# JuliaRobotics/KernelDensityEstimate.jl

Hardware: AMD Instinct MI355X
Metric: gibbs_product_samples_per_sec (higher is better)
Workload: dtype f64

## Files before the change

### kerneldensityestimate.jl_amd/csrc/gibbs_lean.hip

```cpp
#define KDEHIP_EXP256 1
#ifndef KDEHIP_PRELOAD_MAXB
#define KDEHIP_PRELOAD_MAXB 8
#endif
#include "gibbs_device.hpp"
#include "screen_device.hpp"

namespace kdehip {

template <int I> using IC = std::integral_constant<int, I>;
template <int N, int I = 0, typename F>
__device__ __forceinline__ void static_for(F &&f) {
  if constexpr (I < N) {
    f(IC<I>{});
    static_for<N, I + 1>(f);
  }
}

#if defined(KDEHIP_LEAN_HI) || (defined(KDEHIP_LEAN_DEV_M) && KDEHIP_LEAN_DEV_M > 4)
constexpr int kLeanMinDens = 8, kLeanMaxDens = 8;
#else
constexpr int kLeanMinDens = 2, kLeanMaxDens = 4;
#endif
constexpr int kLeanMaxNormals = 128;

__device__ __forceinline__ int scalar_copy(int x) {
  int y;
  asm("s_mov_b32 %0, %1" : "=s"(y) : "s"(x));
  return y;
}

template <int D>
struct LeanTile {
  int n;
  int flags;
  int lds_off;
  int stage_bytes;
  int chunk_rows;
  int seg;
  int hdr_lo, hdr_hi;
  int B, F, last_lane;
  int uniform_bw;
  __device__ __forceinline__ int64_t hdr_off() const {
    return (static_cast<int64_t>(hdr_hi) << 32) | static_cast<uint32_t>(hdr_lo);
  }
  __device__ __forceinline__ void load(const kdehip_v8i &d) {
    n = scalar_copy(d[0]);
    flags = scalar_copy(d[1]);
    lds_off = scalar_copy(d[2]);
    stage_bytes = scalar_copy(d[3]);
    chunk_rows = scalar_copy(d[4]);
    seg = scalar_copy(d[5]);
    hdr_lo = scalar_copy(d[6]);
    hdr_hi = scalar_copy(d[7]);
    B = (n + 63) >> 6;
    last_lane = flags & 0xFF;
    uniform_bw = flags >> 8;
    F = uniform_bw ? D + 1 : 2 * D + 1;
  }
};

template <typename P, typename T, bool OK> constexpr bool kCanPreloadImpl = OK && kIsLdsPtr<P> && sizeof(T) == 8;

template <typename T, int D, int M, int WAVES, bool BATCH = false, bool SCHUNK = false>
__global__ __launch_bounds__(WAVES * 64) void gibbs_lean_kernel(PlanDev plan_, RunArgs a_) {
  const LaunchView<BATCH> view(plan_, a_);
  const PlanDev &plan = view.plan;
  const auto &a = view.a;
  constexpr bool kPrefetchRows = (WAVES <= 12) || sizeof(T) == 4 || D <= 4;
  using RowPtr = std::conditional_t<(WAVES == 16 && sizeof(T) == 8), LdsPtrSplit<T>, LdsPtr<T>>;
  constexpr int kCopyWaves = WAVES > 4 ? 4 : WAVES;
  constexpr bool kKeptRows = (WAVES <= 8);
  constexpr bool kScreen = sizeof(T) == 8 && !BATCH;
  constexpr bool kPreloadBuild = kKeptRows && kPrefetchRows;
  constexpr int kNormOff = 2048;
  constexpr int kUnifOff = kNormOff + WAVES * kLeanMaxNormals * 8;
  constexpr int kPoolOff = kUnifOff + WAVES * 1024;
  constexpr bool kCoop = kScreen && SCHUNK && WAVES == 8;
  constexpr int kXchgOff = kPoolOff + kLdsPoolBytes;
  constexpr int kXchgSlotDoubles = 32 + 4 * 64;
  constexpr int kXchgBytes = kCoop ? 64 + WAVES * kXchgSlotDoubles * 8 : 0;
  static_assert(kPoolOff + kLdsPoolBytes + kXchgBytes <= 160 * 1024, "LDS budget of one CU exceeded");
  __shared__ __attribute__((aligned(1024))) unsigned char smem[kPoolOff + kLdsPoolBytes + kXchgBytes];

  double *sExpTab = reinterpret_cast<double *>(smem);
  if (threadIdx.x < 256) sExpTab[threadIdx.x] = kExp2Tab256[threadIdx.x];
  if constexpr (kCoop) {
    if (threadIdx.x < 16) reinterpret_cast<int *>(smem + kXchgOff)[threadIdx.x] = 0;
  }

  const int lane = threadIdx.x & 63;
  const int wave = __builtin_amdgcn_readfirstlane(static_cast<int>(threadIdx.x >> 6));
  KDEHIP_PRIO_CHAIN();
  const int chain = wave;
  int64_t s = static_cast<int64_t>(view.block) * WAVES + chain;
  const bool live = s < a.Np;
  if (!live) s = a.Np - 1;
  const uint64_t gs = static_cast<uint64_t>(a.sample_offset + s);
  const void *fb = live ? static_cast<const void *>(plan.levels) : nullptr;

  const int L = plan.L;
  const T *__restrict__ data = static_cast<const T *>(plan.data);
  const LevelTable levels{(const __attribute__((address_space(4))) kdehip_v16i *)(plan.levels)};
  const StepTable steps{(const __attribute__((address_space(4))) kdehip_v8i *)(plan.levels + 2 * plan.M * (plan.L + 1))};
  unsigned char *pool = smem + kPoolOff;
  const int dl = lane < D ? lane : D - 1;
  const int vlev = a.variant % 1000;

  double *sNorm = reinterpret_cast<double *>(smem + kNormOff) + chain * kLeanMaxNormals;
  const int R = D * (L + 1);
  if (a.rng_philox) {
    for (int b = lane; 2 * b < R; b += 64) {
      double n0, n1;
      philox_normal_pair(a.seed, gs, static_cast<uint32_t>(b), n0, n1);
      sNorm[2 * b] = n0;
      if (2 * b + 1 < R) sNorm[2 * b + 1] = n1;
    }
  } else {
    for (int r = lane; r < R; r += 64) sNorm[r] = a.randN[s * a.R + r];
  }
  __syncthreads();

  T lam[M], lmu[M];
  int psel[M];

  auto adopt = [&](auto jc, const auto &ds, auto hdr, int pos) {
    constexpr int j = decltype(jc)::value;
    using TA = TileAddr<T>;
    auto e = hdr + kTileHeader + TA::row(pos >> 6, TA::stride(ds.F)) + (pos & 63) * TA::kLane;
    const T mu = e[dl * TA::kField];
    const T var = ds.uniform_bw ? hdr[dl] : e[(D + dl) * TA::kField];
    const T l = fast_rcp(var);
    lam[j] = l;
    lmu[j] = mu * l;
    psel[j] = pos;
  };
  auto product = [&](auto skipc, T &mean, T &cov) {
    constexpr int skip = decltype(skipc)::value;
    T ls = T(0), ms = T(0);
    static_for<M>([&](auto kc) {
      constexpr int k = decltype(kc)::value;
      if constexpr (k != skip) { ls += lam[k]; ms += lmu[k]; }
    });
    cov = fast_rcp(ls);
    mean = cov * ms;
  };

  auto draw = [&](const auto &ds, auto hdr, T mean, T cov, auto &&run) -> int {
    if (ds.uniform_bw) {
      EvalUniform<T, D> ev;
      ev.tab = sExpTab;
      const T c = hdr[dl] + cov;
      T cen, nin;
      EvalUniform<T, D>::operands(mean, c, true, cen, nin);
      T Pr = T(1);
#pragma unroll
      for (int d = 0; d < D; ++d) {
        ev.center[d] = lane_read(cen, d);
        ev.ninv[d] = lane_read(nin, d);
        Pr *= lane_read(c, d);
      }
      ev.scale = Num<T>::rsqrt(Pr);
      return run(ev);
    }
    EvalFast<T, D, false> ev;
    ev.tab = sExpTab;
    ev.act = 0;
#pragma unroll
    for (int d = 0; d < D; ++d) {
      ev.center[d] = lane_read(mean, d);
      ev.cov[d] = lane_read(cov, d);
    }
    return run(ev);
  };

  uint32_t c = static_cast<uint32_t>(M);
  uint32_t ubatch = 0xFFFFFFFFu;
  double *sUnif = reinterpret_cast<double *>(smem + kUnifOff) + wave * 128;
  auto next_uniform = [&]() -> double {
    const uint32_t b = c >> 7;
    if (b != ubatch) {
      ubatch = b;
      double u_even, u_odd;
      if (a.rng_philox) {
        const Philox4 r = philox_block(a.seed, gs, b * 64u + static_cast<uint32_t>(lane), 0u);
        u_even = bits_to_unit(r.v[0], r.v[1]);
        u_odd = bits_to_unit(r.v[2], r.v[3]);
      } else {
        const int64_t i0 = s * a.K + static_cast<int64_t>(b) * 128 + 2 * lane - 1;
        u_even = (i0 >= 0 && i0 < a.nU) ? a.randU[i0] : 0.5;
        u_odd = (i0 + 1 < a.nU) ? a.randU[i0 + 1] : 0.5;
      }
      wave_sync();
      sUnif[2 * lane] = u_even;
      sUnif[2 * lane + 1] = u_odd;
      wave_sync();
    }
    const double u = sUnif[c & 127u];
    ++c;
    return u;
  };

  static_for<M>([&](auto jc) {
    const LevelDesc ds = levels[decltype(jc)::value * (L + 1)];
    adopt(jc, ds, data + ds.hdr_off, 0);
  });

  const TabTable tabs{(const __attribute__((address_space(4))) kdehip_v8i *)(plan.tabdesc)};
  const T *tables = static_cast<const T *>(plan.tables);
  const int Lt = (vlev == 1 || vlev == 4 || !a.use_tables) ? 0 : plan.Lt;

  auto draw_rows = [&](const auto &ds, auto rows, const auto &ev, double u) -> int {
    using P = decltype(rows);
    return draw_label<T, P, kPrefetchRows, kKeptRows>(rows, ds, lane, ev, u, fb);
  };

  auto draw_rows_repeat = [&](const auto &ds, const T *rows, const auto &ev, double u) -> int {
    using Ev = std::decay_t<decltype(ev)>;
    if constexpr (kScreen && SCHUNK && sizeof(typename Ev::Row) <= 7 * sizeof(T) && WAVES <= 8) {
      LaneAcc<T> acc;
      KDEHIP_PRIO_ROWS();
      lane_rows_all_deep<T, Ev>(rows, ds.B, TileAddr<T>::stride(ds.F), lane, ev, acc);
      KDEHIP_PRIO_CHAIN();
      return select_or_raise<T, const T *>(acc.total(), rows, ds, lane, ev, u, fb);
    }
    return draw_rows(ds, rows, ev, u);
  };

#ifdef KDEHIP_SCREEN_STAMPS
  unsigned long long rstamp[8] = {0, 0, 0, 0, 0, 0, 0, 0}, r_prev_end = 0;
  bool rstamp_on = false;
#define RSTAMP(var) const unsigned long long var = __builtin_amdgcn_s_memtime()
#define RSTAMP_ADD(slot, t0, t1) do { if (rstamp_on) rstamp[slot] += (t1) - (t0); } while (0)
#else
#define RSTAMP(var) do {} while (0)
#define RSTAMP_ADD(slot, t0, t1) do {} while (0)
#endif
  auto step_kept = [&](auto jc, const auto &ds, auto hdr, const auto &row, T mean, T cov, double u) {
    RSTAMP(tr1);
    auto rows1 = hdr + kTileHeader;
    using P1 = decltype(rows1);
    using Ev = EvalFast<T, D, false>;
    Ev ev;
    ev.tab = sExpTab;
    ev.act = 0;
#pragma unroll
    for (int d = 0; d < D; ++d) {
      ev.center[d] = lane_read(mean, d);
      ev.cov[d] = lane_read(cov, d);
    }
#ifdef KDEHIP_SCREEN_STAMPS
    asm volatile("" ::"s"(ev.center[D - 1]), "s"(ev.cov[D - 1]));
#endif
    RSTAMP(tr2);
    RSTAMP_ADD(1, tr1, tr2);
    int pos1;
    if (ds.B == 1) {
      const T S = ev(row);
      pos1 = select_or_raise<T, P1>(S, rows1, ds, lane, ev, u, fb);
    } else if (ds.B <= 4) {
      pos1 = draw_label_kept<T, P1, Ev, 4>(rows1, ds, lane, ev, u, fb, row);
    } else {
      pos1 = draw_label_kept<T, P1, Ev, 8>(rows1, ds, lane, ev, u, fb, row);
    }
    pos1 = __builtin_amdgcn_readfirstlane(pos1);
    RSTAMP(tr3);
    RSTAMP_ADD(2, tr2, tr3);
    adopt(jc, ds, hdr, pos1);
#ifdef KDEHIP_SCREEN_STAMPS
    {
      const double sink = lam[decltype(jc)::value] + lmu[decltype(jc)::value];
      asm volatile("" ::"v"(sink));
    }
#endif
    RSTAMP(tr4);
    RSTAMP_ADD(3, tr3, tr4);
#ifdef KDEHIP_SCREEN_STAMPS
    r_prev_end = tr4;
#endif
  };

  auto step = [&](auto jc, const auto &ds, auto hdr, bool first, T x) {
    if constexpr (kCanPreloadImpl<decltype(hdr + kTileHeader), T, kPreloadBuild>) {
      if (!ds.uniform_bw && ds.B <= KDEHIP_PRELOAD_MAXB) {
        RSTAMP(tr0);
#ifdef KDEHIP_SCREEN_STAMPS
        if (r_prev_end) RSTAMP_ADD(4, r_prev_end, tr0);
#endif
        const auto row = EvalFast<T, D, false>().load(hdr + kTileHeader + lane * TileAddr<T>::kLane);
        T mean1 = x, cov1 = T(0);
        if (!first) product(jc, mean1, cov1);
        const double u1 = next_uniform();
#ifdef KDEHIP_SCREEN_STAMPS
        asm volatile("" ::"v"(mean1), "v"(cov1), "v"(u1));
        {
          RSTAMP(trp);
          RSTAMP_ADD(0, tr0, trp);
        }
#endif
        step_kept(jc, ds, hdr, row, mean1, cov1, u1);
        return;
      }
    }
    T mean = x, cov = T(0);
    if (!first) product(jc, mean, cov);
    const double u = next_uniform();
    auto rows = hdr + kTileHeader;
    const int pos = __builtin_amdgcn_readfirstlane(draw(ds, hdr, mean, cov, [&](const auto &ev) {
      return draw_rows(ds, rows, ev, u);
    }));
    adopt(jc, ds, hdr, pos);
  };

  uint32_t n_screened = 0, n_repeated = 0;
#ifdef KDEHIP_SCREEN_STAMPS
  unsigned long long sstamp[8] = {0, 0, 0, 0, 0, 0, 0, 0};
  bool sstamp_on = false;
#endif
  auto screen_eval = [&](const auto &ds, double mu0, double cmin, float mmax, float valid, T mean, T cov, auto &&body) -> int {
    const float cen = static_cast<float>(mean - mu0);
    const float cf = static_cast<float>(cmin + cov), covf = static_cast<float>(cov);
    const float acen = fabsf(cen);
    const float t = fminf(mmax + acen, 2.0f * acen);
    float a2 = lane < D ? t * t * __builtin_amdgcn_rcpf(cf) : 0.0f;
    const bool inr = (acen <= kScreenMaxAbsMean) && (covf <= static_cast<float>(kScreenMaxVar)) && (a2 <= kScreenMaxA2);
    const bool ok = valid != 0.0f && __ballot(lane < D && !inr) == 0ull;
    if (ds.uniform_bw) {
      ScreenEval<D, true> ev;
      ev.a2 = a2; ev.nsum = (ds.B + 1) >> 1;
      const float ninv = -kScreenC0 * __builtin_amdgcn_rcpf(cf);
      float pr = 1.0f;
#pragma unroll
      for (int d = 0; d < D; ++d) {
        ev.cen[d] = lane_read(cen, d);
        ev.b[d] = lane_read(ninv, d);
        pr *= lane_read(cf, d);
      }
      ev.scale = __builtin_amdgcn_rsqf(pr);
      return body(ev, ok);
    } else {
      ScreenEval<D, false> ev;
      ev.a2 = a2; ev.nsum = (ds.B + 1) >> 1; ev.scale = 1.0f;
#pragma unroll
      for (int d = 0; d < D; ++d) {
        ev.cen[d] = lane_read(cen, d);
        ev.b[d] = lane_read(covf, d);
      }
      return body(ev, ok);
    }
  };
  auto screen_finish = [&](auto jc, const auto &ds, int pos, T mean, T cov, double u) {
    const T *hdrg = data + ds.hdr_off();
    ++n_screened;
    if (pos < 0) {
      ++n_repeated;
      pos = __builtin_amdgcn_readfirstlane(draw(ds, hdrg, mean, cov, [&](const auto &ev) {
        return draw_rows_repeat(ds, hdrg + kTileHeader, ev, u);
      }));
    }
    adopt(jc, ds, hdrg, pos);
  };
  bool pend = false;
  T pend_mean = T(0), pend_cov = T(0);
  double pend_u = 0.0;
  int cstep = 0;
  auto coop_post = [&](T mean, T cov, double u) {
    if constexpr (kCoop) {
      pend = true; pend_mean = mean; pend_cov = cov; pend_u = u;
      double *xs = reinterpret_cast<double *>(smem + kXchgOff + 64) + wave * kXchgSlotDoubles;
      if (lane < D) { xs[dl] = static_cast<double>(mean); xs[8 + dl] = static_cast<double>(cov); }
      if (lane == 0) reinterpret_cast<int *>(smem + kXchgOff)[(cstep & 1) * WAVES + wave] = 1;
    }
  };
  auto coop_resolve = [&](auto jp, const auto &dsp, int par) {
    if constexpr (kCoop) {
      int *flags = reinterpret_cast<int *>(smem + kXchgOff) + par * WAVES;
      const int f = flags[lane & (WAVES - 1)];
      const unsigned mask = static_cast<unsigned>(__ballot(f != 0 && lane < WAVES));
      if (mask == 0u) return;
      using TA = TileAddr<T>;
      const T *hdrg = data + dsp.hdr_off();
      const T *rows = hdrg + kTileHeader;
      const int RS = TA::stride(dsp.F), B = dsp.B;
      const int group = wave >> 2, k = wave & 3;
      int idx = 0;
      for (unsigned m = mask; m != 0u; m &= m - 1u, ++idx) {
        if ((idx & 1) != group) continue;
        const int r = __builtin_ctz(m);
        double *xs = reinterpret_cast<double *>(smem + kXchgOff + 64) + r * kXchgSlotDoubles;
        const T mean_r = static_cast<T>(xs[dl]), cov_r = static_cast<T>(xs[8 + dl]);
        T acc = T(0);
        KDEHIP_PRIO_ROWS();
        draw(dsp, hdrg, mean_r, cov_r, [&](const auto &ev) {
          using Ev = std::decay_t<decltype(ev)>;
          using Row = typename Ev::Row;
          const T *e = rows + lane * TA::kLane;
          auto at = [&](int rr) { return e + TA::row(rr < B ? rr : B - 1, RS); };
          if constexpr (sizeof(Row) <= 4 * sizeof(T)) {
            Row a0 = ev.load(at(k)), a1 = ev.load(at(k + 4)), a2 = ev.load(at(k + 8)), a3 = ev.load(at(k + 12));
            int i = k;
            for (; i + 12 < B; i += 16) {
              const Row b0 = ev.load(at(i + 16)), b1 = ev.load(at(i + 20)), b2 = ev.load(at(i + 24)), b3 = ev.load(at(i + 28));
              __builtin_amdgcn_sched_barrier(0);
              acc += ev(a0); acc += ev(a1); acc += ev(a2); acc += ev(a3);
              a0 = b0; a1 = b1; a2 = b2; a3 = b3;
            }
            if (i < B) acc += ev(a0);
            if (i + 4 < B) acc += ev(a1);
            if (i + 8 < B) acc += ev(a2);
          } else {
            Row a0 = ev.load(at(k)), a1 = ev.load(at(k + 4));
            int i = k;
            for (; i + 4 < B; i += 8) {
              const Row b0 = ev.load(at(i + 8)), b1 = ev.load(at(i + 12));
              __builtin_amdgcn_sched_barrier(0);
              acc += ev(a0); acc += ev(a1);
              a0 = b0; a1 = b1;
            }
            if (i < B) acc += ev(a0);
          }
          return 0;
        });
        KDEHIP_PRIO_CHAIN();
        xs[32 + 64 * k + lane] = static_cast<double>(acc);
      }
      __syncthreads();
      if (pend) {
        double *xs = reinterpret_cast<double *>(smem + kXchgOff + 64) + wave * kXchgSlotDoubles;
        const T a0 = static_cast<T>(xs[32 + lane]), a1 = static_cast<T>(xs[32 + 64 + lane]);
        const T a2 = static_cast<T>(xs[32 + 128 + lane]), a3 = static_cast<T>(xs[32 + 192 + lane]);
        const T S = (a0 + a1) + (a2 + a3);
        const int pos = __builtin_amdgcn_readfirstlane(draw(dsp, hdrg, pend_mean, pend_cov, [&](const auto &ev) {
          return select_or_raise<T, const T *>(S, rows, dsp, lane, ev, pend_u, fb);
        }));
        adopt(jp, dsp, hdrg, pos);
        pend = false;
        if (lane == 0) flags[wave] = 0;
      }
    }
  };

  auto step_screen = [&](auto jc, const auto &ds, int sc_lds_off, bool first, T x) {
    if constexpr (kScreen) {
      SSTAMP(ts0);
      const LdsPtr<float> h32 = (LdsPtr<float>)(pool + sc_lds_off);
      const LdsPtr<double> h64 = (LdsPtr<double>)(pool + sc_lds_off);
      const double mu0 = h64[dl], cmin = h64[8 + dl];
      const float mmax = h32[32 + dl], valid = h32[40];
      T mean = x, cov = T(0);
      if (!first) product(jc, mean, cov);
      const double u = next_uniform();
      SSTAMP(ts1);
      SSTAMP_ADD(0, ts0, ts1);
      const float cen = static_cast<float>(mean - mu0);
      const float cf = static_cast<float>(cmin + cov), covf = static_cast<float>(cov);
      const float acen = fabsf(cen);
      const float t = fminf(mmax + acen, 2.0f * acen);
      float a2 = lane < D ? t * t * __builtin_amdgcn_rcpf(cf) : 0.0f;
      const bool inr = (acen <= kScreenMaxAbsMean) && (covf <= static_cast<float>(kScreenMaxVar)) && (a2 <= kScreenMaxA2);
      int pos = -1;
      const T *hdrg = data + ds.hdr_off();
      if (valid != 0.0f && __ballot(lane < D && !inr) == 0ull) {
        const LdsPtr<float> rows32 = h32 + kScreenHeaderFloats;
        if (ds.uniform_bw) {
          ScreenEval<D, true> ev;
          ev.a2 = a2; ev.nsum = (ds.B + 1) >> 1;
          const float ninv = -kScreenC0 * __builtin_amdgcn_rcpf(cf);
          float pr = 1.0f;
#pragma unroll
          for (int d = 0; d < D; ++d) {
            ev.cen[d] = lane_read(cen, d);
            ev.b[d] = lane_read(ninv, d);
            pr *= lane_read(cf, d);
          }
          ev.scale = __builtin_amdgcn_rsqf(pr);
          pos = screen_draw<D, true>(rows32, ds.n, ds.B, ds.F, lane, ev, u SSTAMP_ARGS);
        } else {
          ScreenEval<D, false> ev;
          ev.a2 = a2; ev.nsum = (ds.B + 1) >> 1; ev.scale = 1.0f;
#pragma unroll
          for (int d = 0; d < D; ++d) {
            ev.cen[d] = lane_read(cen, d);
            ev.b[d] = lane_read(covf, d);
          }
          pos = screen_draw<D, false>(rows32, ds.n, ds.B, ds.F, lane, ev, u SSTAMP_ARGS);
        }
        pos = __builtin_amdgcn_readfirstlane(pos);
      }
      SSTAMP(ts2);
      SSTAMP_ADD(1, ts1, ts2);
      ++n_screened;
      if (pos < 0) {
        ++n_repeated;
        pos = __builtin_amdgcn_readfirstlane(draw(ds, hdrg, mean, cov, [&](const auto &ev) {
          return draw_rows_repeat(ds, hdrg + kTileHeader, ev, u);
        }));
      }
      SSTAMP(ts3);
      SSTAMP_ADD(2, ts2, ts3);
      adopt(jc, ds, hdrg, pos);
#ifdef KDEHIP_SCREEN_STAMPS
      {
        const double sink = lam[decltype(jc)::value] + lmu[decltype(jc)::value];
        asm volatile("" ::"v"(sink));
      }
#endif
      SSTAMP(ts4);
      SSTAMP_ADD(3, ts3, ts4);
    }
  };

  int gchunk = 0;
  auto stage_chunk = [&](const auto &ds, int r0, int half) {
    using TA = TileAddr<T>;
    const int RS = TA::stride(ds.F), rc = ds.chunk_rows;
    const int nrows = (ds.B - r0 < rc) ? (ds.B - r0) : rc;
    const int bytes = (static_cast<int>(TA::span(nrows, RS)) * int(sizeof(T)) + 1023) & ~1023;
    const unsigned char *src = reinterpret_cast<const unsigned char *>(data + ds.hdr_off() + kTileHeader + TA::row(r0, RS));
    if (wave < kCopyWaves) stage_tile<kCopyWaves>(src, pool + half * (kLdsPoolBytes / 2), bytes, wave, lane);
  };

  auto stage_schunk = [&](const LevelDesc &sc, int p0, int half) {
    using TA = TileAddr<float>;
    const int RS = TA::stride(sc.F), cp = sc.chunk_rows >> 1, npairs = (sc.B + 1) >> 1;
    const int np = (npairs - p0 < cp) ? (npairs - p0) : cp;
    const int head = p0 == 0 ? kScreenHeaderFloats : 0;
    const int bytes = ((head + np * RS) * 4 + 1023) & ~1023;
    const unsigned char *src = reinterpret_cast<const unsigned char *>(reinterpret_cast<const float *>(plan.data) + sc.hdr_off +
                                                                       (p0 == 0 ? 0 : kScreenHeaderFloats + p0 * RS));
    if (wave < kCopyWaves) stage_tile<kCopyWaves>(src, pool + half * (kLdsPoolBytes / 2), bytes, wave, lane);
  };
  auto step_screen_chunked = [&](auto jc, const auto &ds, const auto &dsp, const LevelDesc &sc, const LevelDesc &scn, bool more,
                                 bool first, bool level_start, T x) {
    if constexpr (kScreen && SCHUNK) {
      using TA = TileAddr<float>;
      T mean = x, cov = T(0);
      const bool was_pend = kCoop && pend;
      if (!first && !was_pend) product(jc, mean, cov);
      const double u = next_uniform();
      const int RS = TA::stride(sc.F), cp = sc.chunk_rows >> 1, npairs = (sc.B + 1) >> 1;
      staging_barrier();
      if (cp < npairs) stage_schunk(sc, cp, (gchunk + 1) & 1);
      else if (more) stage_schunk(scn, 0, (gchunk + 1) & 1);
      if constexpr (kCoop) {
        constexpr int j = decltype(jc)::value;
        if (!level_start) coop_resolve(IC<(j + M - 1) % M>{}, dsp, (cstep + 1) & 1);
        if (was_pend && !first) product(jc, mean, cov);
      }
      const LdsPtr<float> h32 = (LdsPtr<float>)(pool + (gchunk & 1) * (kLdsPoolBytes / 2));
      const LdsPtr<double> h64 = (LdsPtr<double>)(pool + (gchunk & 1) * (kLdsPoolBytes / 2));
      const double mu0 = h64[dl], cmin = h64[8 + dl];
      const float mmax = h32[32 + dl], valid = h32[40];
      const float *grows = reinterpret_cast<const float *>(plan.data) + sc.hdr_off + kScreenHeaderFloats;
      const int pos = __builtin_amdgcn_readfirstlane(screen_eval(ds, mu0, cmin, mmax, valid, mean, cov, [&](const auto &ev, bool ok) {
        using Ev = std::decay_t<decltype(ev)>;
        ScreenSums q;
        KDEHIP_PRIO_ROWS();
        if (ok) screen_rows<D, Ev::kUni>(h32 + kScreenHeaderFloats + lane * TA::kLane, npairs < cp ? npairs : cp, RS, ev, q);
        ++gchunk;
        for (int p0 = cp; p0 < npairs; p0 += cp, ++gchunk) {
          staging_barrier();
          if (p0 + cp < npairs) stage_schunk(sc, p0 + cp, (gchunk + 1) & 1);
          else if (more) stage_schunk(scn, 0, (gchunk + 1) & 1);
          const int np = (npairs - p0 < cp) ? (npairs - p0) : cp;
          if (ok) screen_rows<D, Ev::kUni>((LdsPtr<float>)(pool + (gchunk & 1) * (kLdsPoolBytes / 2)) + lane * TA::kLane, np, RS, ev, q);
        }
        KDEHIP_PRIO_CHAIN();
        if (!ok) return -1;
        return screen_decide<D, Ev::kUni, true>(grows, ds.n, ds.B, RS, lane, ev, u, q.values(), q.moments() SSTAMP_ARGS);
      }));
      if constexpr (kCoop) {
        ++n_screened;
        if (pos < 0) {
          ++n_repeated;
          coop_post(mean, cov, u);
        } else {
          adopt(jc, ds, data + ds.hdr_off(), pos);
        }
        ++cstep;
      } else {
        screen_finish(jc, ds, pos, mean, cov, u);
      }
    }
  };

#ifdef KDEHIP_EXPERIMENTS
  const int Lrun = (vlev >= 100 && vlev - 100 < L) ? vlev - 100 : L;
#else
  const int Lrun = L;
#endif
  for (int l = 1; l <= Lrun; ++l) {
    T x;
    {
      T mean, cov;
      product(IC<-1>{}, mean, cov);
      x = mean + Num<T>::sqrt(cov) * static_cast<T>(sNorm[(l - 1) * D + dl]);
    }
    const int level_mode = scalar_copy(levels[l].stage_mode);
    auto tile_raw = [&](int j) -> kdehip_v8i { return steps.raw(j * (L + 1) + l); };
    auto tile = [&](int j) -> LeanTile<D> {
      LeanTile<D> t;
      t.load(tile_raw(j));
      return t;
    };
    const int mode = vlev == 1 ? int(kStageGlobal) : level_mode;
    const bool tabulated = (l <= Lt);
    const int npass = tabulated ? 1 : a.Niter + 1;

    bool screened = false, screen_streamed = false, screen_chunked = false;
    if constexpr (kScreen) {
      if (a.use_screen && vlev != 1) {
        const int smode = scalar_copy(levels[M * (L + 1) + l].stage_mode);
        screened = smode == kStageScreen;
        screen_streamed = smode == kStageScreenStream;
        if constexpr (SCHUNK) screen_chunked = smode == kStageScreenChunked;
      }
    }
#ifdef KDEHIP_SCREEN_STAMPS
    rstamp_on = (vlev >= 300 && l == vlev - 300) && view.block == 3 && wave == 5;
    r_prev_end = 0;
#endif
    if (screened) {
#ifdef KDEHIP_SCREEN_STAMPS
      sstamp_on = (l == ((vlev >= 200) ? vlev - 200 : L)) && view.block == 3 && wave == 5;
#endif
      auto screen = [&](int j) -> LevelDesc { return levels[(M + j) * (L + 1) + l]; };
      staging_barrier();
      static_for<M>([&](auto jc) {
        const LevelDesc sc = screen(decltype(jc)::value);
        stage_tile<WAVES>(reinterpret_cast<const unsigned char *>(reinterpret_cast<const float *>(plan.data) + sc.hdr_off),
                          pool + sc.lds_off, sc.stage_bytes, wave, lane);
      });
      staging_barrier();
      for (int p = 0; p < npass; ++p)
        static_for<M>([&](auto jc) {
          const LeanTile<D> ds = tile(decltype(jc)::value);
          step_screen(jc, ds, ds.lds_off, p == 0, x);
        });
    } else if (screen_streamed) {
      auto screen = [&](int j) -> LevelDesc { return levels[(M + j) * (L + 1) + l]; };
      auto stage_screen = [&](const LevelDesc &sc, int half, auto wc) {
        constexpr int W = decltype(wc)::value;
        if (wave < W)
          stage_tile<W>(reinterpret_cast<const unsigned char *>(reinterpret_cast<const float *>(plan.data) + sc.hdr_off),
                        pool + half * (kLdsPoolBytes / 2), sc.stage_bytes, wave, lane);
      };
      staging_barrier();
      stage_screen(screen(0), 0, IC<WAVES>{});
      int t = 0;
      const int nsteps = npass * M;
      for (int p = 0; p < npass; ++p)
        static_for<M>([&](auto jc) {
          constexpr int j = decltype(jc)::value;
          constexpr int jn = (j + 1 == M) ? 0 : j + 1;
          const LeanTile<D> ds = tile(j);
          const LevelDesc scn = screen(jn);
          staging_barrier();
          constexpr bool kLateCopy = kCopyWaves < WAVES;
          if (!kLateCopy && t + 1 < nsteps) stage_screen(scn, (t + 1) & 1, IC<WAVES>{});
          step_screen(jc, ds, (t & 1) * (kLdsPoolBytes / 2), p == 0, x);
          if (kLateCopy && t + 1 < nsteps) stage_screen(scn, (t + 1) & 1, IC<kCopyWaves>{});
          ++t;
        });
    } else if (screen_chunked) {
      auto screen = [&](int j) -> LevelDesc { return levels[(M + j) * (L + 1) + l]; };
      staging_barrier();
      stage_schunk(screen(0), 0, gchunk & 1);
      int t = 0;
      const int nsteps = npass * M;
      for (int p = 0; p < npass; ++p)
        static_for<M>([&](auto jc) {
          constexpr int j = decltype(jc)::value;
          constexpr int jn = (j + 1 == M) ? 0 : j + 1;
          constexpr int jp = (j + M - 1) % M;
          const LeanTile<D> ds = tile(j);
          step_screen_chunked(jc, ds, tile(jp), screen(j), screen(jn), t + 1 < nsteps, p == 0, t == 0, x);
          ++t;
        });
      if constexpr (kCoop) {
        __syncthreads();
        coop_resolve(IC<M - 1>{}, tile(M - 1), (cstep + 1) & 1);
      }
    } else if (mode == kStageResident) {
      staging_barrier();
      static_for<M>([&](auto jc) {
        const LeanTile<D> ds = tile(decltype(jc)::value);
        stage_tile<WAVES>(reinterpret_cast<const unsigned char *>(data + ds.hdr_off()), pool + ds.lds_off, ds.stage_bytes, wave, lane);
      });
      staging_barrier();
      for (int p = 0; p < npass; ++p)
        static_for<M>([&](auto jc) {
          const LeanTile<D> ds = tile(decltype(jc)::value);
          step(jc, ds, (RowPtr)(pool + ds.lds_off), p == 0, x);
        });
    } else if (mode == kStageStream) {
      staging_barrier();
      {
        const LeanTile<D> d0 = tile(0);
        stage_tile<WAVES>(reinterpret_cast<const unsigned char *>(data + d0.hdr_off()), pool, d0.stage_bytes, wave, lane);
      }
      int t = 0;
      const int nsteps = npass * M;
      for (int p = 0; p < npass; ++p)
        static_for<M>([&](auto jc) {
          constexpr int j = decltype(jc)::value;
          constexpr int jn = (j + 1 == M) ? 0 : j + 1;
          const LeanTile<D> ds = tile(j);
          const LeanTile<D> dn = tile(jn);
          T mean = x, cov = T(0);
          if (p != 0) product(jc, mean, cov);
          const double u = next_uniform();
          staging_barrier();
          constexpr bool kLateCopy = kCopyWaves < WAVES;
          if (!kLateCopy && t + 1 < nsteps)
            stage_tile<WAVES>(reinterpret_cast<const unsigned char *>(data + dn.hdr_off()),
                              pool + ((t + 1) & 1) * (kLdsPoolBytes / 2), dn.stage_bytes, wave, lane);
          {
            auto hdr = (RowPtr)(pool + (t & 1) * (kLdsPoolBytes / 2));
            auto rows = hdr + kTileHeader;
            const int pos = __builtin_amdgcn_readfirstlane(draw(ds, hdr, mean, cov, [&](const auto &ev) {
              return draw_rows(ds, rows, ev, u);
            }));
            adopt(jc, ds, hdr, pos);
          }
          if (kLateCopy && t + 1 < nsteps && wave < kCopyWaves)
            stage_tile<kCopyWaves>(reinterpret_cast<const unsigned char *>(data + dn.hdr_off()),
                                   pool + ((t + 1) & 1) * (kLdsPoolBytes / 2), dn.stage_bytes, wave, lane);
          ++t;
        });
    } else if (mode == kStageChunked) {
      staging_barrier();
      stage_chunk(tile(0), 0, gchunk & 1);
      int t = 0;
      const int nsteps = npass * M;
      for (int p = 0; p < npass; ++p)
        static_for<M>([&](auto jc) {
          constexpr int j = decltype(jc)::value;
          constexpr int jn = (j + 1 == M) ? 0 : j + 1;
          const LeanTile<D> ds = tile(j);
          const LeanTile<D> dn = tile(jn);
          T mean = x, cov = T(0);
          if (p != 0) product(jc, mean, cov);
          const double u = next_uniform();
          const T *hdr = data + ds.hdr_off();
          const int pos = draw(ds, hdr, mean, cov, [&](const auto &ev) {
            using Ev = std::decay_t<decltype(ev)>;
            const int RS = TileAddr<T>::stride(ds.F), rc = ds.chunk_rows;
            LaneAcc<T> acc;
            SegSums<T> seg;
            const int cps = seg_chunks(ds.seg);
            const bool use_seg = cps != 0;
            int cin = 0;
            KDEHIP_PRIO_ROWS();
            for (int r0 = 0; r0 < ds.B; r0 += rc, ++gchunk) {
              staging_barrier();
              if (r0 + rc < ds.B) stage_chunk(ds, r0 + rc, (gchunk + 1) & 1);
              else if (t + 1 < nsteps) stage_chunk(dn, 0, (gchunk + 1) & 1);
              const int nrows = (ds.B - r0 < rc) ? (ds.B - r0) : rc;
              const auto crows = (RowPtr)(pool + (gchunk & 1) * (kLdsPoolBytes / 2));
              lane_rows_all<T, RowPtr, Ev, kPrefetchRows>(crows, nrows, RS, lane, ev, acc);
              if (use_seg && ++cin == cps) { seg.note(acc.total()); cin = 0; }
            }
            KDEHIP_PRIO_CHAIN();
            const T S = acc.total();
            if (use_seg)
              return __builtin_amdgcn_readfirstlane(
                  select_or_raise_seg<T, const T *>(S, seg, cps * rc, hdr + kTileHeader, ds, lane, ev, u, fb));
            return __builtin_amdgcn_readfirstlane(select_or_raise<T, const T *>(S, hdr + kTileHeader, ds, lane, ev, u, fb));
          });
          adopt(jc, ds, hdr, pos);
          ++t;
        });
    } else {
      for (int p = 0; p < npass; ++p)
        static_for<M>([&](auto jc) {
          const LeanTile<D> ds = tile(decltype(jc)::value);
          step(jc, ds, data + ds.hdr_off(), p == 0, x);
        });
    }

    if (tabulated) {
      TabDesc td[M];
      static_for<M>([&](auto jc) { td[decltype(jc)::value] = tabs[decltype(jc)::value * (L + 1) + l]; });
      uint32_t word = 0;
      static_for<M>([&](auto jc) { word |= static_cast<uint32_t>(psel[decltype(jc)::value]) << td[decltype(jc)::value].shift; });
      word = __builtin_amdgcn_readfirstlane(word);
      for (int p = 1; p <= a.Niter; ++p)
        static_for<M>([&](auto jc) {
          constexpr int j = decltype(jc)::value;
          const TabDesc &tj = td[j];
          const uint32_t cfg = (word & ((1u << tj.shift) - 1u)) | ((word >> (tj.shift + tj.bits)) << tj.shift);
          const T *row = tables + tj.off + static_cast<int64_t>(cfg) * (tj.n + 1);
          const int n = tj.n;
          const T incl = row[lane < n ? lane : n];
          const double u = next_uniform();
          const T total = lane_read(incl, n < 64 ? n : 63);
          int pos;
          if (!(total >= Num<T>::tiny_total())) {
            count_fallback(fb, lane);
            const LeanTile<D> dk = tile(j);
            const T wl = ((LdsPtr<T>)(pool + dk.lds_off) + kTileHeader)[(dk.F - 1) * TileAddr<T>::kField + (n - 1) * TileAddr<T>::kLane];
            int z = n - 1;
            if (wl > T(0)) {
              z = static_cast<int>(ceil(u * static_cast<double>(n))) - 1;
              z = z < 0 ? 0 : (z > n - 1 ? n - 1 : z);
            }
            pos = __builtin_amdgcn_readfirstlane(z);
          } else {
            const T target = static_cast<T>(u) * total;
            unsigned long long hit = __ballot(target <= incl);
            if (n < 64) hit &= (1ull << n) - 1ull;
            pos = hit ? (__ffsll(hit) - 1) : (n - 1);
          }
          word = (word & ~(((1u << tj.bits) - 1u) << tj.shift)) | (static_cast<uint32_t>(pos) << tj.shift);
        });
      static_for<M>([&](auto jc) {
        constexpr int j = decltype(jc)::value;
        const int pk = static_cast<int>((word >> td[j].shift) & ((1u << td[j].bits) - 1u));
        const LeanTile<D> dk = tile(j);
        adopt(jc, dk, (LdsPtr<T>)(pool + dk.lds_off), pk);
      });
    }
    if (a.labels && live && lane == 0) {
      static_for<M>([&](auto jc) {
        constexpr int j = decltype(jc)::value;
        a.labels[(s * M + j) * L + (l - 1)] = plan.perm[levels[j * (L + 1) + l].perm_off + psel[j]];
      });
    }
    if (l == L && live && lane == 0) {
      static_for<M>([&](auto jc) {
        constexpr int j = decltype(jc)::value;
        const int64_t label = static_cast<int64_t>(plan.perm[levels[j * (L + 1) + l].perm_off + psel[j]]) + 1;
        a.indices[s * M + j] = label;
        for (int k = 0; k < a.npeers; ++k) a.peer_indices[k][s * M + j] = label;
      });
    }
  }

#ifdef KDEHIP_SCREEN_STAMPS
  if (view.block == 3 && wave == 5 && lane == 0)
    for (int k = 0; k < 8; ++k) { g_screen_stamps[k] = sstamp[k]; g_screen_stamps[8 + k] = rstamp[k]; }
#endif
  if constexpr (kScreen) {
    if (live && lane == 0 && n_screened != 0u) {
      unsigned long long *cnt = reinterpret_cast<unsigned long long *>(const_cast<LevelDesc *>(plan.levels));
      atomicAdd(cnt - 3, static_cast<unsigned long long>(n_screened));
      if (n_repeated != 0u) atomicAdd(cnt - 2, static_cast<unsigned long long>(n_repeated));
    }
  }
  {
    T mean, cov;
    product(IC<-1>{}, mean, cov);
    T xf = mean;
    if (a.addEntropy) xf = mean + Num<T>::sqrt(cov) * static_cast<T>(sNorm[L * D + dl]);
    if (live && lane < D) {
      a.points[s * D + lane] = static_cast<double>(xf);
      for (int k = 0; k < a.npeers; ++k) a.peer_points[k][s * D + lane] = static_cast<double>(xf);
    }
  }
}


template <typename T, int D, int M, int WAVES>
static void launch_lean_waves(const PlanDev &plan, const RunArgs &args, hipStream_t stream) {
  const int64_t blocks = (args.Np + WAVES - 1) / WAVES;
  if constexpr (sizeof(T) == 8 && WAVES >= 8) {
    if (M == 8 || (plan.screened == 2 && args.use_screen)) {
      hipLaunchKernelGGL((gibbs_lean_kernel<T, D, M, WAVES, false, true>), dim3(static_cast<unsigned>(blocks)), dim3(WAVES * 64),
                         0, stream, plan, args);
      return;
    }
  }
  if constexpr (!(sizeof(T) == 8 && WAVES >= 8 && M == 8))
    hipLaunchKernelGGL((gibbs_lean_kernel<T, D, M, WAVES>), dim3(static_cast<unsigned>(blocks)), dim3(WAVES * 64), 0,
                       stream, plan, args);
}

static int set_geometry(const PlanDev &, RunArgs &args, int) { return lean_waves(args.Np, args.variant); }

template <typename T, int D, int M>
static int launch_lean_m(const PlanDev &plan, const RunArgs &args_in, hipStream_t stream) {
  RunArgs args = args_in;
  const int waves = set_geometry(plan, args, sizeof(T) == 8 ? 64 : 32);
  if (waves == 16) launch_lean_waves<T, D, M, 16>(plan, args, stream);
  else if (waves == 8) launch_lean_waves<T, D, M, 8>(plan, args, stream);
  else launch_lean_waves<T, D, M, 4>(plan, args, stream);
  const hipError_t e = hipGetLastError();
  if (e != hipSuccess)
    return set_error(KDEHIP_ERR_HIP, std::string("kernel launch failed: ") + hipGetErrorString(e));
  return KDEHIP_OK;
}

#ifndef KDEHIP_DIM
#error "compile gibbs_lean.hip with -DKDEHIP_DIM=<1..8>"
#endif
#define KDEHIP_CAT2(a, b) a##b
#define KDEHIP_CAT(a, b) KDEHIP_CAT2(a, b)

template <typename T, int D, int M>
static int launch_lean_m_hi(const PlanDev &plan, const RunArgs &args_in, hipStream_t stream) {
  RunArgs args = args_in;
  const int waves = set_geometry(plan, args, sizeof(T) == 8 ? 64 : 32);
  if (waves == 16) launch_lean_waves<T, D, M, 16>(plan, args, stream);
  else if (waves == 8) launch_lean_waves<T, D, M, 8>(plan, args, stream);
  else return kLeanNotCovered;
  const hipError_t e = hipGetLastError();
  if (e != hipSuccess)
    return set_error(KDEHIP_ERR_HIP, std::string("kernel launch failed: ") + hipGetErrorString(e));
  return KDEHIP_OK;
}

#if !defined(KDEHIP_LEAN_HI) && !defined(KDEHIP_LEAN_F32) && !defined(KDEHIP_LEAN_DEV)
template <int D, int M>
static void launch_lean_batch_m(const PlanDev &plan, const RunArgs &args, hipStream_t stream) {
  constexpr int W = 16;
  hipLaunchKernelGGL((gibbs_lean_kernel<double, D, M, W, true>), dim3(static_cast<unsigned>(args.Np / W)), dim3(W * 64), 0,
                     stream, plan, args);
}
int KDEHIP_CAT(launch_lean_batch_d, KDEHIP_DIM)(int M, const PlanDev &plan, const RunArgs &args, void *stream) {
  constexpr int D = KDEHIP_DIM;
  hipStream_t st = static_cast<hipStream_t>(stream);
  if (args.Np <= 0) return KDEHIP_OK;
  switch (M) {
    case 2: launch_lean_batch_m<D, 2>(plan, args, st); break;
    case 3: launch_lean_batch_m<D, 3>(plan, args, st); break;
    case 4: launch_lean_batch_m<D, 4>(plan, args, st); break;
    default: return set_error(KDEHIP_ERR_UNSUPPORTED, "batched launch: 2..4 densities");
  }
  const hipError_t e = hipGetLastError();
  if (e != hipSuccess) return set_error(KDEHIP_ERR_HIP, std::string("batched kernel launch failed: ") + hipGetErrorString(e));
  return KDEHIP_OK;
}
#endif

#if defined(KDEHIP_LEAN_DEV) && !defined(KDEHIP_LEAN_HI) && !defined(KDEHIP_LEAN_F32)
int KDEHIP_CAT(launch_lean_batch_d, KDEHIP_DIM)(int, const PlanDev &, const RunArgs &, void *) {
  return set_error(KDEHIP_ERR_UNSUPPORTED, "development library: no batched kernels");
}
#endif

#if defined(KDEHIP_SCREEN_STAMPS)
extern "C" int kdehip_debug_read_screen_stamps(unsigned long long *out) {
  return hipMemcpyFromSymbol(out, HIP_SYMBOL(kdehip::g_screen_stamps), sizeof(unsigned long long) * 16) == hipSuccess ? 0 : -5;
}
#endif

#if defined(KDEHIP_LEAN_HI)
#define KDEHIP_LEAN_ENTRY launch_lean_hi_d
#elif defined(KDEHIP_LEAN_F32)
#define KDEHIP_LEAN_ENTRY launch_lean_f32_d
#else
#define KDEHIP_LEAN_ENTRY launch_lean_d
#endif

int KDEHIP_CAT(KDEHIP_LEAN_ENTRY, KDEHIP_DIM)(int precision, int mode, const PlanDev &plan, const RunArgs &args,
                                              void *stream) {
  constexpr int D = KDEHIP_DIM;
  if (mode != kModeFast || args.table_build || plan.M < kLeanMinDens || plan.M > kLeanMaxDens ||
      D * (plan.L + 1) > kLeanMaxNormals)
    return kLeanNotCovered;
  if (args.Np <= 0) return KDEHIP_OK;
  hipStream_t st = static_cast<hipStream_t>(stream);
  const bool f64 = (precision == 64);
#ifdef KDEHIP_LEAN_DEV
#ifndef KDEHIP_LEAN_DEV_M
#define KDEHIP_LEAN_DEV_M 4
#endif
#ifndef KDEHIP_LEAN_DEV_W
#define KDEHIP_LEAN_DEV_W 8
#endif
#ifdef KDEHIP_LEAN_DEV_F32
  using DevT = float;
#else
  using DevT = double;
#endif
  RunArgs dargs = args;
  if (f64 != (sizeof(DevT) == 8) || plan.M != KDEHIP_LEAN_DEV_M ||
      set_geometry(plan, dargs, precision) != KDEHIP_LEAN_DEV_W)
    return kLeanNotCovered;
  launch_lean_waves<DevT, D, KDEHIP_LEAN_DEV_M, KDEHIP_LEAN_DEV_W>(plan, dargs, st);
  return KDEHIP_OK;
#elif defined(KDEHIP_LEAN_HI)
  if (!f64) return kLeanNotCovered;
  return launch_lean_m_hi<double, D, 8>(plan, args, st);
#elif defined(KDEHIP_LEAN_F32)
  if (f64) return kLeanNotCovered;
  switch (plan.M) {
    case 2: return launch_lean_m<float, D, 2>(plan, args, st);
    case 3: return launch_lean_m<float, D, 3>(plan, args, st);
    default: return launch_lean_m<float, D, 4>(plan, args, st);
  }
#else
  if (!f64) return kLeanNotCovered;
  switch (plan.M) {
    case 2: return launch_lean_m<double, D, 2>(plan, args, st);
    case 3: return launch_lean_m<double, D, 3>(plan, args, st);
    default: return launch_lean_m<double, D, 4>(plan, args, st);
  }
#endif
}

}
```

### kerneldensityestimate.jl_amd/csrc/screen_device.hpp

```cpp
#pragma once
#include "gibbs_device.hpp"

namespace kdehip {

#ifdef KDEHIP_SCREEN_STAMPS
static __device__ unsigned long long g_screen_stamps[32];
#define SSTAMP(var) const unsigned long long var = __builtin_amdgcn_s_memtime()
#define SSTAMP_ADD(slot, t0, t1) do { if (sstamp_on) sstamp[slot] += (t1) - (t0); } while (0)
#define SSTAMP_ARGS , sstamp, sstamp_on
#define SSTAMP_PARAMS , unsigned long long *sstamp, bool sstamp_on
#else
#define SSTAMP_ARGS
#define SSTAMP_PARAMS
#define SSTAMP(var) do {} while (0)
#define SSTAMP_ADD(slot, t0, t1) do {} while (0)
#endif

constexpr float kScreenU = 5.9604645e-8f;
constexpr float kScreenC0 = 0.72134752f;
constexpr float kScreenSqrtC0 = 0.84932180f;
constexpr float kScreenLn2 = 0.69314718f;
template <int D>
struct ScreenConst {
  static constexpr int depth = D <= 1 ? 0 : D <= 2 ? 1 : D <= 4 ? 2 : 3;
  static constexpr float kx_uni = 12 + D, kx_node = 16 + 2 * depth + D;
  static constexpr float vc_uni = D + 9, vc_node = (3 * D + 18) / 2;
};
constexpr double kScreenMargin = 2.1;

template <int D, bool UNI>
struct ScreenEval {
  float cen[D];
  float b[D];
  float scale;
  float a2;
  int nsum;
  __device__ __forceinline__ void bound(float &A, float &Bc) const {
    float s = a2;
    s += dpp_fetch<0x111, 0xF>(s);
    s += dpp_fetch<0x112, 0xF>(s);
    s += dpp_fetch<0x114, 0xF>(s);
    const float na = __builtin_sqrtf(lane_read(s, 7)) * (kScreenU * kScreenSqrtC0 * 1.01f);
    using SC = ScreenConst<D>;
    Bc = (kScreenLn2 * 1.01f) * (na + (UNI ? SC::kx_uni : SC::kx_node) * kScreenU);
    A = (kScreenLn2 * 1.01f) * na + (static_cast<float>(nsum + 9) + (UNI ? SC::vc_uni : SC::vc_node)) * kScreenU;
  }
  static constexpr bool kUni = UNI;
  using TA = TileAddr<float>;
  template <typename V, typename LD>
  __device__ __forceinline__ V value(LD &&ld, V &x) const {
    V front;
    if constexpr (UNI) {
      V acc = V(0.0f);
#pragma unroll
      for (int d = 0; d < D; ++d) {
        const V dl = ld(d) - cen[d];
        acc = Num<V>::fma(dl * dl, V(b[d]), acc);
      }
      front = ld(D) * scale;
      x = acc;
    } else {
      V c[D], d2[D];
#pragma unroll
      for (int d = 0; d < D; ++d) {
        c[d] = ld(D + d) + b[d];
        const V dl = ld(d) - cen[d];
        d2[d] = dl * dl;
      }
      V num, prod;
      fraction_sum<V, 0, D>(d2, c, num, prod);
      const V r = Num<V>::rsqrt(prod);
      const V q = num * r * r;
      front = ld(2 * D) * r;
      x = q * V(-kScreenC0);
    }
    return front * Num<V>::exp_fast(x, nullptr);
  }
  static constexpr int kFields = UNI ? D + 1 : 2 * D + 1;
  struct Pair { kdehip_f2 f[kFields]; };
  static __device__ __forceinline__ Pair load(LdsPtr<float> e) {
    Pair r;
#pragma unroll
    for (int f = 0; f < kFields; ++f) r.f[f] = load_pair(e + f * TA::kField);
    return r;
  }
  __device__ __forceinline__ kdehip_f2 pair(const Pair &r, kdehip_f2 &S, kdehip_f2 &X) const {
    kdehip_f2 x;
    const kdehip_f2 v = value<kdehip_f2>([&](int f) { return r.f[f]; }, x);
    S += v;
    X = Num<kdehip_f2>::fma(v, -x, X);
    return v;
  }
  template <typename P>
  __device__ __forceinline__ float one(P e) const {
    float x;
    return value<float>([&](int f) { return e[f * TA::kField]; }, x);
  }
};

struct ScreenSums {
  kdehip_f2 S = {0.0f, 0.0f}, X = {0.0f, 0.0f};
  __device__ __forceinline__ float values() const { return S.x + S.y; }
  __device__ __forceinline__ float moments() const { return X.x + X.y; }
};
template <int D, bool UNI>
__device__ __forceinline__ void screen_rows(LdsPtr<float> e, int npairs, int RS, const ScreenEval<D, UNI> &ev, ScreenSums &q) {
  using Ev = ScreenEval<D, UNI>;
  typename Ev::Pair ra = Ev::load(e);
  int p = 0;
  if constexpr (UNI && D > 4) {
    const int last = npairs - 1;
    auto at = [&](int k) { return e + (k < last ? k : last) * RS; };
    typename Ev::Pair rb = Ev::load(at(1));
    for (; p + 3 <= npairs; p += 3) {
      const typename Ev::Pair rc = Ev::load(at(p + 2));
      __builtin_amdgcn_sched_barrier(0);
      ev.pair(ra, q.S, q.X);
      ra = Ev::load(at(p + 3));
      __builtin_amdgcn_sched_barrier(0);
      ev.pair(rb, q.S, q.X);
      rb = Ev::load(at(p + 4));
      __builtin_amdgcn_sched_barrier(0);
      ev.pair(rc, q.S, q.X);
    }
    if (p < npairs) ev.pair(ra, q.S, q.X);
    if (p + 1 < npairs) ev.pair(rb, q.S, q.X);
  } else {
    for (; p + 2 <= npairs; p += 2) {
      const typename Ev::Pair rb = Ev::load(e + RS);
      __builtin_amdgcn_sched_barrier(0);
      ev.pair(ra, q.S, q.X);
      e += (p + 2 < npairs) ? 2 * RS : RS;
      ra = Ev::load(e);
      __builtin_amdgcn_sched_barrier(0);
      ev.pair(rb, q.S, q.X);
    }
    if (p < npairs) ev.pair(ra, q.S, q.X);
  }
}

template <int D, bool UNI, bool TWO, typename P>
__device__ __forceinline__ int screen_decide(P rows, int n, int B, int RS, int lane, const ScreenEval<D, UNI> &ev, double u,
                                             float s1, float x1 SSTAMP_PARAMS) {
  using TA = TileAddr<float>;
  SSTAMP(tq1);
  const float incl = wave_inclusive_scan(s1);
  const float xinc = wave_inclusive_scan(x1);
  float A, Bc;
  ev.bound(A, Bc);
  const float total = lane_read(incl, 63), etot = fmaf(A, total, Bc * lane_read(xinc, 63));
  if (!(total >= 0x1p-40f && total < 0x1p100f)) return -1;
  const double td = u * static_cast<double>(total), md = kScreenMargin * static_cast<double>(etot);
  const double id = static_cast<double>(incl);
  const unsigned long long hitA = __ballot(td + md <= id), hitB = __ballot(td - md <= id);
  if (hitA == 0ull) return -1;
  const int lstar = __ffsll(hitA) - 1;
  if (__ffsll(hitB) - 1 != lstar) return -1;
  SSTAMP(tq2);
  SSTAMP_ADD(5, tq1, tq2);
  const float base = lstar > 0 ? lane_read(incl, lstar - 1) : 0.0f;
  int len = n - lstar * B;
  if (len > B) len = B;
  const bool in = lane < len;
  float p2 = 0.0f;
  if (in) p2 = ev.one(rows + lstar * TA::kLane + TA::row(lane, RS));
  const float inc3 = wave_inclusive_scan(p2);
  const double cum = static_cast<double>(base) + static_cast<double>(inc3);
  const unsigned long long hitA2 = __ballot(in && td + md <= cum), hitB2 = __ballot(in && td - md <= cum);
  if constexpr (TWO) {
    if (len > 64) {
      const bool in2 = lane + 64 < len;
      float p3 = 0.0f;
      if (in2) p3 = ev.one(rows + lstar * TA::kLane + TA::row(lane + 64, RS));
      const float inc4 = wave_inclusive_scan(p3);
      const double cum2 = static_cast<double>(base) + static_cast<double>(lane_read(inc3, 63)) + static_cast<double>(inc4);
      const unsigned long long hitA3 = __ballot(in2 && td + md <= cum2), hitB3 = __ballot(in2 && td - md <= cum2);
      const int ia = hitA2 ? __ffsll(hitA2) - 1 : (hitA3 ? 64 + __ffsll(hitA3) - 1 : -1);
      const int ib = hitB2 ? __ffsll(hitB2) - 1 : (hitB3 ? 64 + __ffsll(hitB3) - 1 : -1);
      if (ia < 0 || ia != ib) return -1;
      return ia * 64 + lstar;
    }
  }
  if (hitA2 == 0ull) return -1;
  const int istar = __ffsll(hitA2) - 1;
  if (__ffsll(hitB2) - 1 != istar) return -1;
  SSTAMP(tq3);
  SSTAMP_ADD(6, tq2, tq3);
  return istar * 64 + lstar;
}

template <int D, bool UNI>
__device__ __forceinline__ int screen_draw(LdsPtr<float> rows, int n, int B, int F, int lane, const ScreenEval<D, UNI> &ev,
                                           double u SSTAMP_PARAMS) {
  using TA = TileAddr<float>;
  const int RS = TA::stride(F);
  SSTAMP(tq0);
  ScreenSums q;
  KDEHIP_PRIO_ROWS();
  screen_rows<D, UNI>(rows + lane * TA::kLane, (B + 1) >> 1, RS, ev, q);
  KDEHIP_PRIO_CHAIN();
  const float s1 = q.values(), x1 = q.moments();
#ifdef KDEHIP_SCREEN_STAMPS
  asm volatile("" ::"v"(s1), "v"(x1));
#endif
  SSTAMP(tq1);
  SSTAMP_ADD(4, tq0, tq1);
  return screen_decide<D, UNI, false>(rows, n, B, RS, lane, ev, u, s1, x1 SSTAMP_ARGS);
}

}
```

Baseline: 4.357 million.

## Restructure screen row loop with paired evaluation, partial LDS waits, and hoisted bound

Reworks the screening row loop so uniform-kernel tiles are processed four rows at a time. Pairs of rows are evaluated jointly, and explicit partial lgkmcnt waits let the next loads stay in flight while earlier rows are computed. Node (non-uniform) tiles now use the three-deep prefetch path as well. The bound computation, which needs cross-lane reductions, moves to the start of the row loop so it overlaps with the outstanding LDS loads instead of sitting on the decide path. The cost is higher register pressure and hand-coded waitcnt encodings that depend on the ISA.

New measurement: 4.380 million, median of 6. Within noise of the previous version (+0.5%).

```diff
diff --git a/kerneldensityestimate.jl_amd/csrc/gibbs_lean.hip b/kerneldensityestimate.jl_amd/csrc/gibbs_lean.hip
--- a/kerneldensityestimate.jl_amd/csrc/gibbs_lean.hip
+++ b/kerneldensityestimate.jl_amd/csrc/gibbs_lean.hip
@@ -554,19 +554,20 @@
       const int pos = __builtin_amdgcn_readfirstlane(screen_eval(ds, mu0, cmin, mmax, valid, mean, cov, [&](const auto &ev, bool ok) {
         using Ev = std::decay_t<decltype(ev)>;
         ScreenSums q;
+        ScreenBound bd;
         KDEHIP_PRIO_ROWS();
-        if (ok) screen_rows<D, Ev::kUni>(h32 + kScreenHeaderFloats + lane * TA::kLane, npairs < cp ? npairs : cp, RS, ev, q);
+        if (ok) screen_rows<D, Ev::kUni, true>(h32 + kScreenHeaderFloats + lane * TA::kLane, npairs < cp ? npairs : cp, RS, ev, q, bd);
         ++gchunk;
         for (int p0 = cp; p0 < npairs; p0 += cp, ++gchunk) {
           staging_barrier();
           if (p0 + cp < npairs) stage_schunk(sc, p0 + cp, (gchunk + 1) & 1);
           else if (more) stage_schunk(scn, 0, (gchunk + 1) & 1);
           const int np = (npairs - p0 < cp) ? (npairs - p0) : cp;
-          if (ok) screen_rows<D, Ev::kUni>((LdsPtr<float>)(pool + (gchunk & 1) * (kLdsPoolBytes / 2)) + lane * TA::kLane, np, RS, ev, q);
+          if (ok) screen_rows<D, Ev::kUni, false>((LdsPtr<float>)(pool + (gchunk & 1) * (kLdsPoolBytes / 2)) + lane * TA::kLane, np, RS, ev, q, bd);
         }
         KDEHIP_PRIO_CHAIN();
         if (!ok) return -1;
-        return screen_decide<D, Ev::kUni, true>(grows, ds.n, ds.B, RS, lane, ev, u, q.values(), q.moments() SSTAMP_ARGS);
+        return screen_decide<D, Ev::kUni, true>(grows, ds.n, ds.B, RS, lane, ev, u, q.values(), q.moments(), bd SSTAMP_ARGS);
       }));
       if constexpr (kCoop) {
         ++n_screened;
diff --git a/kerneldensityestimate.jl_amd/csrc/screen_device.hpp b/kerneldensityestimate.jl_amd/csrc/screen_device.hpp
--- a/kerneldensityestimate.jl_amd/csrc/screen_device.hpp
+++ b/kerneldensityestimate.jl_amd/csrc/screen_device.hpp
@@ -91,6 +91,23 @@
     X = Num<kdehip_f2>::fma(v, -x, X);
     return v;
   }
+  __device__ __forceinline__ void pair2(const Pair &ra, const Pair &rb, kdehip_f2 &S, kdehip_f2 &X) const {
+    static_assert(UNI, "the joint evaluation is written for shared-bandwidth tiles");
+    using V = kdehip_f2;
+    V xa = V(0.0f), xb = V(0.0f);
+#pragma unroll
+    for (int d = 0; d < D; ++d) {
+      const V da = ra.f[d] - cen[d], db = rb.f[d] - cen[d];
+      xa = Num<V>::fma(da * da, V(b[d]), xa);
+      xb = Num<V>::fma(db * db, V(b[d]), xb);
+    }
+    const V fa = ra.f[D] * scale, fb = rb.f[D] * scale;
+    const V va = fa * Num<V>::exp_fast(xa, nullptr), vb = fb * Num<V>::exp_fast(xb, nullptr);
+    S += va;
+    X = Num<V>::fma(va, -xa, X);
+    S += vb;
+    X = Num<V>::fma(vb, -xb, X);
+  }
   template <typename P>
   __device__ __forceinline__ float one(P e) const {
     float x;
@@ -103,29 +120,74 @@
   __device__ __forceinline__ float values() const { return S.x + S.y; }
   __device__ __forceinline__ float moments() const { return X.x + X.y; }
 };
+template <int N>
+__device__ __forceinline__ void lds_landed_but() {
+  static_assert(N >= 0 && N <= 15, "lgkmcnt is a 4-bit counter");
+  __builtin_amdgcn_s_waitcnt(0xC07F | (N << 8));
+}
+struct ScreenBound { float A = 0.0f, Bc = 0.0f; };
 template <int D, bool UNI>
-__device__ __forceinline__ void screen_rows(LdsPtr<float> e, int npairs, int RS, const ScreenEval<D, UNI> &ev, ScreenSums &q) {
+__device__ __forceinline__ void screen_bound_here(const ScreenEval<D, UNI> &ev, ScreenBound &bd) {
+  ev.bound(bd.A, bd.Bc);
+  asm volatile("" : "+v"(bd.A), "+v"(bd.Bc));
+}
+template <int D, bool UNI, bool BOUND>
+__device__ __forceinline__ void screen_rows(LdsPtr<float> e, int npairs, int RS, const ScreenEval<D, UNI> &ev, ScreenSums &q,
+                                            ScreenBound &bd) {
   using Ev = ScreenEval<D, UNI>;
   typename Ev::Pair ra = Ev::load(e);
   int p = 0;
-  if constexpr (UNI && D > 4) {
+  if constexpr (!UNI || D > 4) {
     const int last = npairs - 1;
     auto at = [&](int k) { return e + (k < last ? k : last) * RS; };
     typename Ev::Pair rb = Ev::load(at(1));
-    for (; p + 3 <= npairs; p += 3) {
-      const typename Ev::Pair rc = Ev::load(at(p + 2));
-      __builtin_amdgcn_sched_barrier(0);
-      ev.pair(ra, q.S, q.X);
-      ra = Ev::load(at(p + 3));
-      __builtin_amdgcn_sched_barrier(0);
-      ev.pair(rb, q.S, q.X);
-      rb = Ev::load(at(p + 4));
-      __builtin_amdgcn_sched_barrier(0);
-      ev.pair(rc, q.S, q.X);
-    }
-    if (p < npairs) ev.pair(ra, q.S, q.X);
-    if (p + 1 < npairs) ev.pair(rb, q.S, q.X);
+    if constexpr (BOUND) {
+      __builtin_amdgcn_sched_barrier(0);
+      screen_bound_here(ev, bd);
+    }
+    if constexpr (UNI) {
+      constexpr int kGroup = 2 * Ev::kFields < 15 ? 2 * Ev::kFields : 15;
+      for (; p + 4 <= npairs; p += 4) {
+        const typename Ev::Pair rc = Ev::load(at(p + 2)), rd = Ev::load(at(p + 3));
+        __builtin_amdgcn_sched_barrier(0);
+        lds_landed_but<kGroup>();
+        __builtin_amdgcn_sched_barrier(0);
+        ev.pair2(ra, rb, q.S, q.X);
+        __builtin_amdgcn_sched_barrier(0);
+        ra = Ev::load(at(p + 4));
+        rb = Ev::load(at(p + 5));
+        __builtin_amdgcn_sched_barrier(0);
+        lds_landed_but<kGroup>();
+        __builtin_amdgcn_sched_barrier(0);
+        ev.pair2(rc, rd, q.S, q.X);
+      }
+      if (p < npairs) {
+        const typename Ev::Pair rc = Ev::load(at(p + 2));
+        __builtin_amdgcn_sched_barrier(0);
+        ev.pair(ra, q.S, q.X);
+        if (p + 1 < npairs) ev.pair(rb, q.S, q.X);
+        if (p + 2 < npairs) ev.pair(rc, q.S, q.X);
+      }
+    } else {
+      for (; p + 3 <= npairs; p += 3) {
+        const typename Ev::Pair rc = Ev::load(at(p + 2));
+        __builtin_amdgcn_sched_barrier(0);
+        ev.pair(ra, q.S, q.X);
+        ev.pair(rb, q.S, q.X);
+        __builtin_amdgcn_sched_barrier(0);
+        ra = Ev::load(at(p + 3));
+        rb = Ev::load(at(p + 4));
+        __builtin_amdgcn_sched_barrier(0);
+        ev.pair(rc, q.S, q.X);
+      }
+      if (p < npairs) ev.pair(ra, q.S, q.X);
+      if (p + 1 < npairs) ev.pair(rb, q.S, q.X);
+    }
   } else {
+    if constexpr (BOUND) {
+      __builtin_amdgcn_sched_barrier(0);
+      screen_bound_here(ev, bd);
+    }
     for (; p + 2 <= npairs; p += 2) {
       const typename Ev::Pair rb = Ev::load(e + RS);
       __builtin_amdgcn_sched_barrier(0);
@@ -141,13 +203,12 @@
 
 template <int D, bool UNI, bool TWO, typename P>
 __device__ __forceinline__ int screen_decide(P rows, int n, int B, int RS, int lane, const ScreenEval<D, UNI> &ev, double u,
-                                             float s1, float x1 SSTAMP_PARAMS) {
+                                             float s1, float x1, const ScreenBound &bd SSTAMP_PARAMS) {
   using TA = TileAddr<float>;
   SSTAMP(tq1);
   const float incl = wave_inclusive_scan(s1);
   const float xinc = wave_inclusive_scan(x1);
-  float A, Bc;
-  ev.bound(A, Bc);
+  const float A = bd.A, Bc = bd.Bc;
   const float total = lane_read(incl, 63), etot = fmaf(A, total, Bc * lane_read(xinc, 63));
   if (!(total >= 0x1p-40f && total < 0x1p100f)) return -1;
   const double td = u * static_cast<double>(total), md = kScreenMargin * static_cast<double>(etot);
@@ -196,8 +257,9 @@
   const int RS = TA::stride(F);
   SSTAMP(tq0);
   ScreenSums q;
+  ScreenBound bd;
   KDEHIP_PRIO_ROWS();
-  screen_rows<D, UNI>(rows + lane * TA::kLane, (B + 1) >> 1, RS, ev, q);
+  screen_rows<D, UNI, true>(rows + lane * TA::kLane, (B + 1) >> 1, RS, ev, q, bd);
   KDEHIP_PRIO_CHAIN();
   const float s1 = q.values(), x1 = q.moments();
 #ifdef KDEHIP_SCREEN_STAMPS
@@ -205,7 +267,7 @@
 #endif
   SSTAMP(tq1);
   SSTAMP_ADD(4, tq0, tq1);
-  return screen_decide<D, UNI, false>(rows, n, B, RS, lane, ev, u, s1, x1 SSTAMP_ARGS);
-}
-
-}
+  return screen_decide<D, UNI, false>(rows, n, B, RS, lane, ev, u, s1, x1, bd SSTAMP_ARGS);
+}
+
+}
```
